# google/libultrahdr

Hardware: AMD Instinct MI355X
Metric: Mpixels/s encode+decode (API-1 P010+YUV420, 4K), device-resident round trip (higher is better)
Workload: dtype f32; 1 GPU; API-1 3840x2160 round trip per step: encode (P010 HLG + YCbCr420 -> two-pass 3-ch gain map at scale 1, FDCT q95, Huffman: two JPEG scans) + decode (Huffman, IDCT, applyGainMap -> RGBA_F16 linear); frames resident in HBM

## Files before the change

libultrahdr_amd/csrc/api_context.cpp:

```cpp
#include "api_internal.h"

#include <sys/mman.h>
#include <mutex>
#include <algorithm>

namespace uhdr_api {
uhdr_error_info_t ensure(DeviceBuf& b, size_t bytes) {
  if (b.cap >= bytes) return ok_status();
  if (b.p) (void)hipFree(b.p);
  b.p = nullptr;
  b.cap = 0;
  size_t want = bytes + (bytes >> 3) + 256;
  HIP_TRY(hipMalloc(&b.p, want));
  b.cap = want;
  return ok_status();
}


size_t bytes_per_sample(int fmt) {
  switch (fmt) {
    case UHDR_IMG_FMT_24bppYCbCrP010:
    case UHDR_IMG_FMT_30bppYCbCr444: return 2;
    case UHDR_IMG_FMT_24bppRGB888: return 3;
    case UHDR_IMG_FMT_32bppRGBA8888:
// ... 484 lines not shown
  if (c->tab_cap[slot] < bytes) {
    HIP_TRY(hipStreamSynchronize(c->stream));
    if (c->h_tab[slot]) (void)hipHostFree(c->h_tab[slot]);
    if (c->d_tab[slot]) (void)hipFree(c->d_tab[slot]);
    c->h_tab[slot] = nullptr; c->d_tab[slot] = nullptr; c->tab_cap[slot] = 0;
    HIP_TRY(hipHostMalloc((void**)&c->h_tab[slot], bytes, hipHostMallocDefault));
    HIP_TRY(hipMalloc((void**)&c->d_tab[slot], bytes));
    if (!c->tab_ev[slot]) HIP_TRY(hipEventCreateWithFlags(&c->tab_ev[slot], hipEventDisableTiming));
    c->tab_cap[slot] = bytes;
  }
  memcpy(c->h_tab[slot], t.data(), bytes);
  HIP_TRY(hipMemcpyAsync(c->d_tab[slot], c->h_tab[slot], bytes, hipMemcpyHostToDevice, c->stream));
  HIP_TRY(hipEventRecord(c->tab_ev[slot], c->stream));
  c->tab_key[slot] = key;
  *d_out = c->d_tab[slot];
  return ok_status();
}
}


const char* uhdr_hip_version(void) { return "libuhdr_hip 0.3 (gfx950; reference libultrahdr 2.0.2 hot path)"; }

int uhdr_hip_device_count(void) {
  int n = 0;
  if (hipGetDeviceCount(&n) != hipSuccess) return 0;
  return n;
}

int uhdr_hip_current_device(void) {
  int d = -1;
  if (hipGetDevice(&d) != hipSuccess) return -1;
  return d;
}

uhdr_hip_ctx_t* uhdr_hip_create(int device, uhdr_error_info_t* err) {
  auto fail = [&](const char* what, hipError_t e) -> uhdr_hip_ctx_t* {
    if (err) *err = err_status(UHDR_CODEC_ERROR, "uhdr_hip_create: %s failed: %s (no CPU fallback exists behind this library)",
                               what, hipGetErrorString(e));
    return nullptr;
  };
  if (err) *err = ok_status();
  int n = 0;
  hipError_t e = hipGetDeviceCount(&n);
  if (e != hipSuccess || n == 0) return fail("hipGetDeviceCount", e == hipSuccess ? hipErrorNoDevice : e);
  if (device < 0) {
    e = hipGetDevice(&device);
    if (e != hipSuccess) return fail("hipGetDevice", e);
  }
  if (device >= n) return fail("device index", hipErrorInvalidDevice);
  e = hipSetDevice(device);
  if (e != hipSuccess) return fail("hipSetDevice", e);
  uhdr_hip_ctx* c = new uhdr_hip_ctx();
  c->device = device;
  e = hipStreamCreateWithFlags(&c->own_stream, hipStreamNonBlocking);
  if (e != hipSuccess) { delete c; return fail("hipStreamCreate", e); }
  c->stream = c->own_stream;
  uhdr_error_info_t st = upload_lut(&c->d_srgb, host::srgb_inv_oetf_lut(), c->stream);
  if (st.error_code != UHDR_CODEC_OK) {
    if (err) *err = st;
    (void)hipStreamDestroy(c->own_stream);
    delete c;
    return nullptr;
  }
  return c;
}

void uhdr_hip_destroy(uhdr_hip_ctx_t* c) {
  if (!c) return;
  (void)hipSetDevice(c->device);
  (void)hipStreamSynchronize(c->stream);
  for (auto& e : c->prof_entries) { (void)hipEventDestroy(e.a); (void)hipEventDestroy(e.b); }
  float* luts[] = {c->d_srgb, c->d_hlg_inv, c->d_pq_inv, c->d_hlg_oetf, c->d_pq_oetf, c->d_hlg_inv_ootf, (float*)c->d_math,
                   c->d_hlg_buckets, c->d_pq_buckets, c->d_hlg_buckets_pre, c->d_pq_buckets_pre};
  for (float* p : luts) if (p) (void)hipFree(p);
  for (int i = 0; i < kTableSlots; i++) {
    if (c->h_tab[i]) (void)hipHostFree(c->h_tab[i]);
    if (c->d_tab[i]) (void)hipFree(c->d_tab[i]);
    if (c->tab_ev[i]) (void)hipEventDestroy(c->tab_ev[i]);
  }
  for (auto& b : c->scratch) if (b.p) (void)hipFree(b.p);
  for (auto& b : c->jpg) if (b.p) (void)hipFree(b.p);
  for (auto& b : c->enc) if (b.p) (void)hipFree(b.p);
  for (auto& r : c->resident) if (r.buf.p) (void)hipFree(r.buf.p);
  if (c->pending.buf.p) (void)hipFree(c->pending.buf.p);
  if (c->pending.tmp.p) (void)hipFree(c->pending.tmp.p);
  if (c->minmax.p) (void)hipFree(c->minmax.p);
  if (c->d_coef_src) (void)hipFree(c->d_coef_src);
  if (c->d_huff) (void)hipFree(c->d_huff);
  if (c->d_srgb8) (void)hipFree(c->d_srgb8);
  for (float* q : c->d_lin10) if (q) (void)hipFree(q);
  for (auto& g : c->gain_tabs) if (g.d) (void)hipFree(g.d);
  uhdr_hip_comm_destroy(c);
  aux_worker_destroy(c);
  if (c->aux) uhdr_hip_destroy(c->aux);
  if (c->exchange.p) (void)hipFree(c->exchange.p);
  if (c->affine.p) (void)hipFree(c->affine.p);
  if (c->d_srgb_of_byte) (void)hipFree(c->d_srgb_of_byte);
  if (c->h_mm) (void)hipHostFree(c->h_mm);
  if (c->aux_ev) (void)hipEventDestroy(c->aux_ev);
  if (c->aux_ev2) (void)hipEventDestroy(c->aux_ev2);
  if (c->md_ev) (void)hipEventDestroy(c->md_ev);
  if (c->md_stream) (void)hipStreamDestroy(c->md_stream);
  if (c->h_flags) (void)hipHostFree(c->h_flags);
  if (c->pin.p) (void)hipHostFree(c->pin.p);
  if (c->pin.ev) (void)hipEventDestroy(c->pin.ev);
  if (c->huff_tabs.dev.p) (void)hipFree(c->huff_tabs.dev.p);
  if (c->own_stream) (void)hipStreamDestroy(c->own_stream);
  delete c;
}

int uhdr_hip_recycle(uhdr_hip_ctx_t* c, size_t keep_bytes) {
  if (!c) return -1;
  (void)hipSetDevice(c->device);
  (void)hipStreamSynchronize(c->stream);
  uhdr_hip_resident_forget(c);
  uhdr_hip_resident_begin(c);
  uhdr_hip_resident_end(c);
  c->sticky = ok_status();
  for (auto& h : c->huff_hint) h = uhdr_hip_ctx::HuffHint();
  c->stats = uhdr_hip_stats_t();
  c->deferred_md.valid = false;
  std::vector<DeviceBuf*> bufs;
  for (auto& b : c->scratch) bufs.push_back(&b);
  for (auto& b : c->jpg) bufs.push_back(&b);
  for (auto& b : c->enc) bufs.push_back(&b);
  for (auto& r : c->resident) bufs.push_back(&r.buf);
  bufs.push_back(&c->pending.buf);
  bufs.push_back(&c->pending.tmp);
  size_t total = c->pin.cap;
  for (DeviceBuf* b : bufs) total += b->p ? b->cap : 0;
  std::sort(bufs.begin(), bufs.end(), [](const DeviceBuf* a, const DeviceBuf* b) { return (a->p ? a->cap : 0) > (b->p ? b->cap : 0); });
  for (DeviceBuf* b : bufs) {
    if (total <= keep_bytes) break;
    if (!b->p) continue;
    (void)hipFree(b->p);
    total -= b->cap;
    b->p = nullptr;
    b->cap = 0;
  }
  if (total > keep_bytes && c->pin.p) {
    if (c->pin.ev_pending && c->pin.ev) (void)hipEventSynchronize(c->pin.ev);
    (void)hipHostFree(c->pin.p);
    c->pin.p = nullptr;
    c->pin.cap = c->pin.off = 0;
    c->pin.ev_pending = false;
  }
  if (c->aux) (void)uhdr_hip_recycle(c->aux, keep_bytes);
  return c->device;
}

uhdr_error_info_t uhdr_hip_set_stream(uhdr_hip_ctx_t* c, void* hip_stream) {
  if (!c) return err_status(UHDR_CODEC_INVALID_PARAM, "received nullptr for uhdr_hip context");
  HIP_TRY(hipStreamSynchronize(c->stream));
  c->stream = hip_stream ? (hipStream_t)hip_stream : c->own_stream;
  return ok_status();
}

void* uhdr_hip_get_stream(uhdr_hip_ctx_t* c) { return c ? (void*)c->stream : nullptr; }

uhdr_error_info_t uhdr_hip_synchronize(uhdr_hip_ctx_t* c) {
  if (!c) return err_status(UHDR_CODEC_INVALID_PARAM, "received nullptr for uhdr_hip context");
  HIP_TRY(hipStreamSynchronize(c->stream));
  return ok_status();
}

void uhdr_hip_get_stats(uhdr_hip_ctx_t* c, uhdr_hip_stats_t* out) {
  if (!out) return;
  if (!c) { memset(out, 0, sizeof *out); return; }
  *out = c->stats;
}

namespace {
std::mutex g_seam_mu;
std::vector<uhdr_hip_seam_stage_t> g_seam_rows;
unsigned long long g_seam_seq = 0;
void seam_dump_at_exit() {
  const char* path = getenv("UHDR_HIP_SEAM_STATS_FILE");
  FILE* f = path ? fopen(path, "w") : nullptr;
// ... 176 lines not shown
```

libultrahdr_amd/csrc/api_entropy.cpp:

```cpp
#include "api_internal.h"

#include <condition_variable>
#include <functional>
#include <mutex>

uhdr_error_info_t uhdr_api::check_scan(const uhdr_hip_jpeg_scan_t* sc, bool need_coef, int* mcus_per_row, int* mcu_rows, int* blocks_per_mcu) {
  if (!sc) return err_status(UHDR_CODEC_INVALID_PARAM, "received nullptr for the scan description");
  if (sc->num_components != 1 && sc->num_components != 3)
    return err_status(UHDR_CODEC_INVALID_PARAM, "a scan has 1 or 3 components, received %d", sc->num_components);
  if (sc->w == 0 || sc->h == 0 || sc->w > 65535 || sc->h > 65535)
    return err_status(UHDR_CODEC_INVALID_PARAM, "image dimensions %ux%u are outside JPEG's 1..65535", sc->w, sc->h);
  int hmax = 1, vmax = 1, bpm = 0;
  for (int i = 0; i < sc->num_components; i++) {
    const int hs = sc->num_components == 1 ? 1 : sc->h_samp[i], vs = sc->num_components == 1 ? 1 : sc->v_samp[i];
    if (hs < 1 || hs > 2 || vs < 1 || vs > 2) return err_status(UHDR_CODEC_INVALID_PARAM, "component %d: sampling factors %dx%d not in {1, 2}", i, hs, vs);
    if (hs > hmax) hmax = hs;
    if (vs > vmax) vmax = vs;
    bpm += hs * vs;
    if (need_coef && (!sc->coef[i] || ((uintptr_t)sc->coef[i] & 15)))
      return err_status(UHDR_CODEC_INVALID_PARAM, "coefficient buffer %d is null or not 16-byte aligned", i);
    if (sc->blocks_w[i] < 1 || sc->blocks_h[i] < 1) return err_status(UHDR_CODEC_INVALID_PARAM, "component %d: empty block grid", i);
  }
  if (sc->num_components == 1) {
    *mcus_per_row = sc->blocks_w[0];
// ... 32 lines not shown


uhdr_error_info_t uhdr_hip_huffman_encode_dev(uhdr_hip_ctx_t* c, const uhdr_hip_jpeg_scan_t* sc, uint8_t* out, size_t out_capacity,
                                              size_t* out_bytes) {
  if (!c) return err_status(UHDR_CODEC_INVALID_PARAM, "received nullptr for uhdr_hip context");
  if (!out || !out_bytes) return err_status(UHDR_CODEC_INVALID_PARAM, "received nullptr for the output buffer or size");
  int mpr = 0, mrows = 0, bpm = 0;
  UHDR_TRY(check_scan(sc, true, &mpr, &mrows, &bpm));
  const bool stream = sc->restart_interval == 0;
  if (!stream && (sc->restart_interval < 1 || sc->restart_interval > 65535 || sc->restart_interval * bpm > 64))
    return err_status(UHDR_CODEC_UNSUPPORTED_FEATURE, "restart_interval must be 0 (no markers) or in 1..%d for %d blocks per MCU (one wavefront "
                      "encodes one restart interval of at most 64 blocks); received %d", 64 / bpm, bpm, sc->restart_interval);
  if (stream && 2 * bpm > 64) return err_status(UHDR_CODEC_UNSUPPORTED_FEATURE, "%d blocks per MCU: outside the HIP path", bpm);
  HIP_TRY(hipSetDevice(c->device));
  if (!c->d_huff) {
    std::vector<uint32_t> blob(host::jpeg_huff_code_tables());
    blob.resize((size_t)host::kHuffTabWords + 16);
    memcpy(blob.data() + host::kHuffTabWords, host::jpeg_zigzag_to_natural(), 64);
    HIP_TRY(hipMalloc((void**)&c->d_huff, blob.size() * sizeof(uint32_t)));
    HIP_TRY(hipMemcpyAsync(c->d_huff, blob.data(), blob.size() * sizeof(uint32_t), hipMemcpyHostToDevice, c->stream));
    HIP_TRY(hipStreamSynchronize(c->stream));
  }
  HuffArgs a;
  memset(&a, 0, sizeof a);
  a.ncomp = sc->num_components;
  for (int i = 0; i < a.ncomp; i++) {
    a.coef[i] = sc->coef[i];
    a.bw[i] = sc->blocks_w[i]; a.bh[i] = sc->blocks_h[i];
    a.hs[i] = a.ncomp == 1 ? 1 : sc->h_samp[i]; a.vs[i] = a.ncomp == 1 ? 1 : sc->v_samp[i];
  }
  a.mcus_per_row = mpr;
  a.total_mcus = mpr * mrows;
  a.ri = stream ? huff_stream_segment_mcus(bpm) : sc->restart_interval;
  a.blocks_per_mcu = bpm;
  a.nseg = (a.total_mcus + a.ri - 1) / a.ri;
  a.tables = c->d_huff;
  a.zigzag = (const uint8_t*)(c->d_huff + host::kHuffTabWords);
  if (stream) {
    if (out_capacity > 0xFFFFFFF0u) out_capacity = 0xFFFFFFF0u;
    HuffStream t;
    memset(&t, 0, sizeof t);
    t.raw_words = ((uint64_t)out_capacity + 3) / 4 + 1;
    const uint64_t worst_words = (uint64_t)a.total_mcus * bpm * 52 + 2;
    if (t.raw_words > worst_words) t.raw_words = worst_words;
    const int nchunks = huff_stuff_chunks(t.raw_words * 4u);
    UHDR_TRY(ensure(c->scratch[4], (size_t)t.raw_words * 4));
    UHDR_TRY(ensure(c->scratch[5], ((size_t)a.nseg + 2) * sizeof(uint64_t) + (4 + (size_t)a.nseg + (size_t)nchunks) * sizeof(uint32_t)));
    t.raw = (uint32_t*)c->scratch[4].p;
    t.seg_start = (uint64_t*)c->scratch[5].p;
    uint64_t* d_total = t.seg_start + (size_t)a.nseg + 1;
    t.meta = (uint32_t*)(d_total + 1);
    t.seg_bits = t.meta + 4;
    uint32_t* chunk_counts = t.seg_bits + a.nseg;
    {
      ProfScope ps(c, "huffman_encode");
      HIP_TRY(launch_huffman_encode_stream(a, t, chunk_counts, d_total, out, (uint64_t)out_capacity, c->stream));
    }
    c->stats.entropy_encode_stream++;
    if (!c->h_flags) HIP_TRY(hipHostMalloc((void**)&c->h_flags, 64 * sizeof(uint32_t), hipHostMallocDefault));
    uint32_t* hp = c->h_flags + 48;
    HIP_TRY(hipMemcpyAsync(hp, d_total, sizeof(uint64_t) + 4 * sizeof(uint32_t), hipMemcpyDeviceToHost, c->stream));
    HIP_TRY(wait_stream(c));
    uint64_t total = 0;
    uint32_t meta[4] = {0, 0, 0, 0};
    memcpy(&total, hp, sizeof total);
    memcpy(meta, hp + 2, sizeof meta);
    if (meta[2]) return err_status(UHDR_CODEC_INVALID_PARAM, "coefficients outside the baseline range (DC difference beyond 11 bits / AC beyond 10 bits)");
    const uint64_t raw_bytes = ((((uint64_t)meta[1] << 32) | meta[0]) + 7) / 8;
    if (raw_bytes > t.raw_words * 4u) total = raw_bytes + raw_bytes / 64 + 64;
    *out_bytes = (size_t)total;
    if (total > out_capacity)
      return err_status(UHDR_CODEC_MEM_ERROR, "entropy-coded data needs %llu bytes, the output buffer holds %zu", (unsigned long long)total, out_capacity);
    return ok_status();
  }
  a.slot_stride = huff_slot_stride();
  UHDR_TRY(ensure(c->scratch[4], (size_t)a.nseg * a.slot_stride));
  const size_t meta = (size_t)a.nseg * sizeof(uint32_t) + 16 + ((size_t)a.nseg + 1) * sizeof(uint64_t) + 16;
  UHDR_TRY(ensure(c->scratch[5], meta));
  a.slots = (uint8_t*)c->scratch[4].p;
  uint64_t* offsets = (uint64_t*)c->scratch[5].p;
  uint32_t* status = (uint32_t*)(offsets + (size_t)a.nseg + 1);
  a.seg_bytes = status + 2;
  {
    ProfScope ps(c, "huffman_encode");
    HIP_TRY(launch_huffman_encode(a, offsets, status, out, (uint64_t)out_capacity, c->stream));
  }
  c->stats.entropy_encode_intervals++;
  uint64_t total = 0;
  uint32_t bad = 0;
  HIP_TRY(hipMemcpyAsync(&total, offsets + a.nseg, sizeof total, hipMemcpyDeviceToHost, c->stream));
  HIP_TRY(hipMemcpyAsync(&bad, status, sizeof bad, hipMemcpyDeviceToHost, c->stream));
  HIP_TRY(wait_stream(c));
  if (bad) return err_status(UHDR_CODEC_INVALID_PARAM, "coefficients outside the baseline range (DC difference beyond 11 bits / AC beyond 10 bits)");
  *out_bytes = (size_t)total;
  if (total > out_capacity)
    return err_status(UHDR_CODEC_MEM_ERROR, "entropy-coded data needs %llu bytes, the output buffer holds %zu", (unsigned long long)total, out_capacity);
  return ok_status();
}

static bool make_dec_table(const uint8_t bits[17], const uint8_t vals[256], HuffDecTable* t) {
  memset(t, 0, sizeof *t);
  int nsym = 0;
  for (int l = 1; l <= 16; l++) nsym += bits[l];
  if (nsym > 256) return false;
  int code = 0, k = 0;
  for (int l = 1; l <= 16; l++) {
// ... 508 lines not shown
      if (settled && rst_sync && ((fl[1] & 14u) != 0 || fl[9] != (uint32_t)(a.nseg - 1) || fl[0] != fl[16] || fl[7] != fl[17])) {
        for (int i = 0; i < a.ncomp; i++) HIP_TRY(hipMemsetAsync(a.coef[i], 0, zero_bytes[i], c->stream));
        coef_zeroed = true;
      } else if (settled) {
        if (fl[1] & 8u) return err_status(UHDR_CODEC_INVALID_PARAM, "corrupt entropy-coded data (the scan ends before its last block)");
        if (fl[1] & 2u) return err_status(UHDR_CODEC_INVALID_PARAM, "corrupt entropy-coded data (undefined Huffman code or a run past the end of a block)");
        sync_done = true;
      } else {
        if (a.nseg == 1 && !c->huff_serial_ok && data_bytes > (256u << 10)) {
          c->stats.entropy_decode_declined++;
          return err_status(UHDR_CODEC_UNSUPPORTED_FEATURE, "the parallel entropy decode did not settle in %d rounds; %zu bytes on one lane would take longer than the CPU", max_rounds, data_bytes);
        }
        for (int i = 0; i < a.ncomp; i++) HIP_TRY(hipMemsetAsync(a.coef[i], 0, zero_bytes[i], c->stream));
        coef_zeroed = true;
      }
    }
  }
  if (sync_done) {
    c->stats.entropy_decode_parallel++;
    return ok_status();
  }
  if (a.nseg == 1 && !c->huff_serial_ok && data_bytes > (256u << 10)) {
    c->stats.entropy_decode_declined++;
    return err_status(UHDR_CODEC_UNSUPPORTED_FEATURE, "a %zu-byte scan without restart markers that the parallel decoder does not take (Huffman tables outside its two-level form)", data_bytes);
  }
  if (!coef_zeroed)
    for (int i = 0; i < a.ncomp; i++) HIP_TRY(hipMemsetAsync(a.coef[i], 0, zero_bytes[i], c->stream));
  HIP_TRY(hipMemsetAsync(a.status, 0, 16, c->stream));
  {
    ProfScope ps(c, "huffman_decode");
    HIP_TRY(launch_huffman_decode(a, counts, starts, ends, c->stream));
  }
  if (a.nseg == 1) c->stats.entropy_decode_single_lane++;
  else c->stats.entropy_decode_intervals++;
  uint32_t st[2] = {0, 0};
  HIP_TRY(hipMemcpyAsync(st, a.status, sizeof st, hipMemcpyDeviceToHost, c->stream));
  HIP_TRY(wait_stream(c));
  if (st[1] != (uint32_t)(a.nseg - 1))
    return err_status(UHDR_CODEC_INVALID_PARAM, "found %u restart markers, a restart interval of %d MCUs over %d MCUs needs %d", st[1], a.ri,
                      a.total_mcus, a.nseg - 1);
  if (st[0] & 4u) return err_status(UHDR_CODEC_INVALID_PARAM, "restart markers out of sequence");
  if (st[0] & 2u) return err_status(UHDR_CODEC_INVALID_PARAM, "corrupt entropy-coded data (undefined Huffman code or a run past the end of a block)");
  return ok_status();
}

uhdr_error_info_t uhdr_api::aux_context(uhdr_hip_ctx* c, uhdr_hip_ctx** out) {
  if (!c->aux) {
    uhdr_error_info_t e = ok_status();
    c->aux = uhdr_hip_create(c->device, &e);
    if (!c->aux) return e.error_code != UHDR_CODEC_OK ? e : err_status(UHDR_CODEC_ERROR, "could not create the auxiliary context");
  }
  c->aux->prof = c->prof;
  c->aux->huff_serial_ok = c->huff_serial_ok;
  *out = c->aux;
  return ok_status();
}
void uhdr_api::aux_merge(uhdr_hip_ctx* c) {
  if (!c->aux) return;
  uhdr_hip_ctx* x = c->aux;
  c->stats.entropy_decode_parallel += x->stats.entropy_decode_parallel;
  c->stats.entropy_decode_intervals += x->stats.entropy_decode_intervals;
  c->stats.entropy_decode_single_lane += x->stats.entropy_decode_single_lane;
  c->stats.entropy_decode_declined += x->stats.entropy_decode_declined;
  c->stats.entropy_encode_stream += x->stats.entropy_encode_stream;
  c->stats.entropy_encode_intervals += x->stats.entropy_encode_intervals;
  x->stats = uhdr_hip_stats_t();
  for (auto& e : x->prof_entries) c->prof_entries.push_back(e);
  x->prof_entries.clear();
}

struct AuxWorker {
  static constexpr int kSpinUs = 300;
  std::thread th;
  std::mutex mu;
  std::condition_variable cv;
  std::function<void()> job;
  std::atomic<int> state{0};
  std::atomic<bool> busy{false};
  static bool spin_until(const std::function<bool()>& pred, int us) {
    const auto t0 = std::chrono::steady_clock::now();
    while (!pred()) {
      if (std::chrono::steady_clock::now() - t0 > std::chrono::microseconds(us)) return pred();
#if defined(__x86_64__)
      __builtin_ia32_pause();
#endif
    }
    return true;
  }
  AuxWorker() {
    th = std::thread([this] {
      for (;;) {
        if (!spin_until([this] { return state.load(std::memory_order_acquire) != 0; }, kSpinUs)) {
          std::unique_lock<std::mutex> lk(mu);
          cv.wait(lk, [this] { return state.load(std::memory_order_acquire) != 0; });
        }
        if (state.load(std::memory_order_acquire) == 2) return;
        std::function<void()> j;
        {
          std::lock_guard<std::mutex> lk(mu);
          j = std::move(job);
          state.store(0, std::memory_order_release);
        }
        j();
        {
          std::lock_guard<std::mutex> lk(mu);
          busy.store(false, std::memory_order_release);
// ... 108 lines not shown
```

libultrahdr_amd/csrc/api_internal.h:

```cpp
#ifndef UHDR_HIP_API_INTERNAL_H
#define UHDR_HIP_API_INTERNAL_H

#pragma GCC visibility push(default)
#include "uhdr_hip.h"
#pragma GCC visibility pop

#include <cfloat>
#include <chrono>
#include <cmath>
#include <cstdarg>
#include <cstdio>
#include <cstring>
#include <atomic>
#include <functional>
#include <map>
#include <memory>
#include <string>
#include <thread>
#include <vector>
#include "exact_math.h"
#include "host_tables.h"
#include "uhdr_types.h"
#include "rccl_bind.h"

// ... 24 lines not shown
                        "HIP error '%s' at %s:%d", hipGetErrorString(e_), __FILE__, __LINE__); \
  } while (0)
#define UHDR_TRY(expr)                                 \
  do {                                                 \
    uhdr_error_info_t s_ = (expr);                     \
    if (s_.error_code != UHDR_CODEC_OK) return s_;     \
  } while (0)

struct DbgClock {
  bool on;
  std::chrono::steady_clock::time_point t0;
  DbgClock() : on(getenv("UHDR_HIP_CLOCK_DEBUG") != nullptr), t0(std::chrono::steady_clock::now()) {}
  void mark(const char* what) const {
    if (on) fprintf(stderr, "uhdr_hip:   [%7.1f us] %s\n", std::chrono::duration<double, std::micro>(std::chrono::steady_clock::now() - t0).count(), what);
  }
};

struct ProfEntry {
  hipEvent_t a, b;
  std::string family;
};

constexpr int kTableSlots = 4;

struct DeviceBuf {
  void* p = nullptr;
  size_t cap = 0;
};

struct uhdr_hip_ctx {
  int device = 0;
  hipStream_t own_stream = nullptr;
  hipStream_t stream = nullptr;
  float* d_srgb = nullptr;
  float* d_hlg_inv = nullptr;
  float* d_pq_inv = nullptr;
  float* d_hlg_oetf = nullptr;
  float* d_pq_oetf = nullptr;
  float* d_hlg_buckets = nullptr;
  float* d_pq_buckets = nullptr;
  float* d_hlg_buckets_pre = nullptr;
  float* d_pq_buckets_pre = nullptr;
  float* d_hlg_inv_ootf = nullptr;
  double* d_math = nullptr;
  float* h_tab[kTableSlots] = {};
  float* d_tab[kTableSlots] = {};
  size_t tab_cap[kTableSlots] = {};
  hipEvent_t tab_ev[kTableSlots] = {};
  std::string tab_key[kTableSlots];
  int tab_next = 0;
  DeviceBuf scratch[8];
  uhdr_hip_stats_t stats = {};
  bool huff_serial_ok = true;
  DeviceBuf enc[3];
  uhdr_hip_ctx* aux = nullptr;
  struct AuxWorker* aux_worker = nullptr;
  DeviceBuf jpg[6];
  struct Resident {
    DeviceBuf buf;
    bool valid = false;
    uhdr_img_fmt_t fmt = UHDR_IMG_FMT_UNSPECIFIED;
    unsigned int w = 0, h = 0;
    const void* host[3] = {};
    unsigned int host_stride[3] = {};
    size_t off[3] = {};
    unsigned int dev_stride[3] = {};
    unsigned int prows[3] = {}, pcols[3] = {};
    bool host_unwritten = false;
    bool adopted = false;
    void* adopt_dst = nullptr;
    unsigned int adopt_stride = 0, adopt_w = 0, adopt_h = 0;
    bool adopt_expand = false;
  } resident[2];
  struct HuffHint { uint32_t sub_bits = 0, bits_per_block = 0; } huff_hint[16];
  struct HuffTabCache {
    bool valid = false, fast_ok = false;
    uint8_t key[4 * (17 + 256)] = {};
    DeviceBuf dev;
  } huff_tabs;
  struct PinArena {
    void* p = nullptr;
    size_t cap = 0, off = 0;
    hipEvent_t ev = nullptr;
    bool ev_pending = false;
  } pin;
  uint32_t* h_flags = nullptr;
  bool resident_on = false;
  bool resident_lazy = false;
  uhdr_error_info_t sticky = {};
  unsigned int resident_next = 0;
  struct PendingCopy {
    DeviceBuf buf;
    bool on = false;
    size_t off = 0, pitch = 0, dst_pitch = 0;
    unsigned int w = 0, h = 0, bps = 0;
    bool expand = false;
    void* dst = nullptr;
    DeviceBuf tmp;
  } pending;
  struct MallEntry { const void* p; uint64_t stamp; };
  std::vector<MallEntry> mall;
  uint64_t mall_clock = 0;
  DeviceBuf minmax;
  uint32_t* d_huff = nullptr;
  CoefSrc* d_coef_src = nullptr;
  unsigned int coef_src_next = 0;
// ... 94 lines not shown
```

libultrahdr_amd/csrc/huffman_encode.hip:

```cpp
#include "lds_copy.h"
#include "wg_scan.h"
#include "uhdr_types.h"

namespace uhdr {
namespace {

constexpr int kSegBlocks = 64;
constexpr int kWordsPerBlock = 52;
constexpr int kCoefRow = 33;

__device__ __forceinline__ uint32_t wave_incl_scan(uint32_t v, uint32_t lane) {
#pragma unroll
  for (int d = 1; d < 64; d <<= 1) {
    const uint32_t y = (uint32_t)__shfl_up((int)v, d, 64);
    if (lane >= (uint32_t)d) v += y;
  }
  return v;
}

__device__ __forceinline__ uint64_t zigzag_nonzero_map(const uint32_t* s_coef, uint32_t zz_of_lane, uint32_t lane) {
  uint64_t mine = 0;
  const uint32_t word = zz_of_lane >> 1, sh = (zz_of_lane & 1u) * 16u;
#pragma unroll 4
  for (uint32_t b = 0; b < (uint32_t)kSegBlocks; b++) {
// ... 316 lines not shown
      else pred = s_dc[(int)lane - bpm + hs * vs - 1];
    }
    const uint32_t* dct = s_tab + (c ? (16 + 256) : 0);
    const uint32_t* act = dct + 16;
    const int diff = dcv - pred;
    const uint64_t nz = zigzag_nonzero_map(s_coef, s_zz[lane], lane);
    uint32_t len = 0, oob = 0;
    if (emits) walk_block(dct, act, diff, real, crow, s_zz, nz, oob, [&](uint32_t, uint32_t n) { len += n; });
    const uint32_t incl = wave_incl_scan(len, lane);
    const uint32_t total_bits = (uint32_t)__shfl((int)incl, 63, 64);
    if constexpr (PASS == 0) {
      const bool bad = __builtin_amdgcn_ballot_w64(oob != 0) != 0;
      if (lane == 0) t.seg_bits[seg] = bad ? kBadCoef : total_bits;
    } else {
      const uint32_t phase = (uint32_t)(start & 31u);
      if (phase + total_bits > kCapBits) continue;
      const uint32_t nwords = (phase + total_bits + 31u) >> 5;
      for (uint32_t i = lane; i < nwords + 1u; i += 64) s_bits[i] = 0u;
      __syncthreads();
      if (emits) {
        const uint32_t off = phase + incl - len;
        uint64_t acc = 0;
        uint32_t cnt = off & 31u, w = off >> 5;
        walk_block(dct, act, diff, real, crow, s_zz, nz, oob, [&](uint32_t code, uint32_t n) {
          acc = (acc << n) | (uint64_t)code;
          cnt += n;
          if (cnt >= 32u) {
            cnt -= 32u;
            atomicOr(&s_bits[w++], (uint32_t)(acc >> cnt));
          }
        });
        if (cnt) atomicOr(&s_bits[w], (uint32_t)(acc << (32u - cnt)));
      }
      __syncthreads();
      const uint64_t end_bit = start + total_bits;
      if (seg == a.nseg - 1 && lane == 0 && (end_bit & 7u)) {
        const uint32_t e = phase + total_bits, pad = 8u - (e & 7u), pos = e & 31u;
        s_bits[e >> 5] |= ((1u << pad) - 1u) << (32u - pos - pad);
      }
      __syncthreads();
      const uint64_t w0 = start >> 5;
      const uint32_t tail = (phase + total_bits) & 31u;
      for (uint32_t i = lane; i < nwords; i += 64) {
        if (w0 + i >= t.raw_words) break;
        const uint32_t v = __builtin_bswap32(s_bits[i]);
        const bool shared = (i == 0 && phase != 0) || (i == nwords - 1 && tail != 0);
        if (shared) atomicOr(&t.raw[w0 + i], v);
        else t.raw[w0 + i] = v;
      }
    }
  }
}

template <int NT = 1024, typename Sink>
__device__ __forceinline__ uint64_t wg_scan_tiles(const uint32_t* __restrict__ v, int n, uint32_t* s_val , uint64_t* s_sum , Sink sink) {
  const int tid = (int)threadIdx.x;
  uint64_t carry = 0;
  for (int base = 0; base < n; base += 8 * NT) {
    uint32_t ld[8];
#pragma unroll
    for (int j = 0; j < 8; j++) ld[j] = v[min(base + j * NT + tid, n - 1)];
#pragma unroll
    for (int j = 0; j < 8; j++) s_val[j * NT + tid] = base + j * NT + tid < n ? ld[j] : 0u;
    __syncthreads();
    uint32_t x[8];
    uint64_t sum = 0;
#pragma unroll
    for (int j = 0; j < 8; j++) { x[j] = s_val[tid * 8 + j]; sum += x[j]; }
    uint64_t sc[1] = {sum}, all[1];
    wg_incl_scan<NT, 1>(sc, s_sum, all);
    uint64_t run = carry + sc[0] - sum;
#pragma unroll
    for (int j = 0; j < 8; j++) {
      const int i = base + tid * 8 + j;
      if (i < n) sink(i, x[j], run);
      run += x[j];
    }
    carry += all[0];
  }
  return carry;
}

constexpr int kStreamScanThreads = 256;
__global__ __launch_bounds__(kStreamScanThreads) void huff_stream_scan_kernel(const uint32_t* __restrict__ seg_bits, int nseg, const HuffStream t) {
  __shared__ uint32_t s_val[8 * kStreamScanThreads];
  __shared__ uint64_t s_sum[kStreamScanThreads / 64];
  __shared__ uint32_t s_bad;
  const int tid = (int)threadIdx.x;
  if (tid == 0) s_bad = 0;
  __syncthreads();
  bool bad = false;
  uint32_t big = 0;
  const uint64_t total = wg_scan_tiles<kStreamScanThreads>(seg_bits, nseg, s_val, s_sum, [&](int i, uint32_t n, uint64_t run) {
    bad |= n >= kRetry;
    big += (n < kRetry && n + 32u > (uint32_t)(kSegBlocks * kWordsSmall) * 32u) ? 1u : 0u;
    t.seg_start[i] = run;
    if ((run >> 5) < t.raw_words) t.raw[run >> 5] = 0u;
  });
  if (bad) atomicOr(&s_bad, 1u);
  if (big) atomicAdd(&s_bad, big << 1);
  __syncthreads();
  if (tid == kStreamScanThreads - 1) {
    t.seg_start[nseg] = total;
    if ((total >> 5) < t.raw_words) t.raw[total >> 5] = 0u;
    t.meta[0] = (uint32_t)total;
    t.meta[1] = (uint32_t)(total >> 32);
// ... 55 lines not shown
  if ((uint64_t)blockIdx.x * kStuffChunk >= nraw) return;
  const uint64_t base = (uint64_t)blockIdx.x * kStuffChunk + threadIdx.x * 16u;
  uint4 v = make_uint4(0, 0, 0, 0);
  uint32_t nv = 0;
  if (base < nraw) {
    v = raw_load16(t, base);
    nv = (uint32_t)min((uint64_t)16, nraw - base);
  }
  const uint32_t mask = ff_mask16(v, nv), nff = (uint32_t)__builtin_popcount(mask);
  const uint32_t lane = threadIdx.x & 63, wv = threadIdx.x >> 6;
  const uint32_t incl = wave_incl_scan(nff, lane);
  if (lane == 63) s_wave[wv] = incl;
  __syncthreads();
  uint32_t before = chunk_base[blockIdx.x] + incl - nff;
  for (uint32_t k = 0; k < wv; k++) before += s_wave[k];
  uint64_t pos = base + before;
  if (mask == 0 && nv == 16 && pos + 16 <= cap) {
    uint8_t* d = out + pos;
    __builtin_memcpy(d, &v.x, 4);
    __builtin_memcpy(d + 4, &v.y, 4);
    __builtin_memcpy(d + 8, &v.z, 4);
    __builtin_memcpy(d + 12, &v.w, 4);
    return;
  }
  const uint32_t w[4] = {v.x, v.y, v.z, v.w};
  for (uint32_t k = 0; k < nv; k++) {
    const uint32_t b = (w[k >> 2] >> (8u * (k & 3u))) & 0xffu;
    if (pos < cap) out[pos] = (uint8_t)b;
    pos++;
    if (b == 0xffu) {
      if (pos < cap) out[pos] = 0;
      pos++;
    }
  }
}

}

uint32_t huff_slot_stride() { return (uint32_t)(kSegBlocks * kWordsPerBlock * 4 * 2); }

hipError_t launch_huffman_encode(const HuffArgs& a, uint64_t* offsets, uint32_t* status, uint8_t* out, uint64_t cap, hipStream_t s) {
  int grid = a.nseg < 8192 ? a.nseg : 8192;
  const int per = a.ri * a.blocks_per_mcu, groups = per > 32 ? 1 : 64 / per;
  const int nwseg = (a.nseg + groups - 1) / groups;
  hipLaunchKernelGGL((huff_encode_kernel<kWordsSmall, false>), dim3(nwseg < 8192 ? nwseg : 8192), dim3(64), 0, s, a);
  hipLaunchKernelGGL((huff_encode_kernel<kWordsPerBlock, true>), dim3(grid < 2048 ? grid : 2048), dim3(64), 0, s, a);
  hipLaunchKernelGGL(huff_offsets_kernel, dim3(1), dim3(1024), 0, s, a.seg_bytes, a.nseg, offsets, status);
  hipLaunchKernelGGL(huff_gather_kernel, dim3(grid), dim3(256), 0, s, a.slots, a.slot_stride, a.seg_bytes, offsets, a.nseg, out, cap);
  return hipGetLastError();
}


int huff_stream_segment_mcus(int blocks_per_mcu) { return kSegBlocks / blocks_per_mcu - 1; }
int huff_stuff_chunks(uint64_t raw_bytes) { return (int)((raw_bytes + kStuffChunk - 1) / kStuffChunk); }

hipError_t launch_huffman_encode_stream(const HuffArgs& a, const HuffStream& t, uint32_t* chunk_counts, uint64_t* out_bytes, uint8_t* out, uint64_t cap,
                                        hipStream_t s) {
  const int grid = a.nseg < 16384 ? a.nseg : 16384;
  const int nchunks = huff_stuff_chunks(t.raw_words * 4u);
  hipLaunchKernelGGL((huff_stream_kernel<1, 0>), dim3(grid), dim3(64), 0, s, a, t);
  hipLaunchKernelGGL(huff_stream_scan_kernel, dim3(1), dim3(kStreamScanThreads), 0, s, (const uint32_t*)t.seg_bits, a.nseg, t);
  hipLaunchKernelGGL((huff_stream_kernel<kWordsSmall, 1>), dim3(grid), dim3(64), 0, s, a, t);
  hipLaunchKernelGGL((huff_stream_kernel<kWordsPerBlock, 2>), dim3(grid < 2048 ? grid : 2048), dim3(64), 0, s, a, t);
  hipLaunchKernelGGL(huff_stuff_count_kernel, dim3(nchunks), dim3(256), 0, s, t, chunk_counts);
  hipLaunchKernelGGL(huff_stuff_scan_kernel, dim3(1), dim3(kStreamScanThreads), 0, s, chunk_counts, nchunks, t, out_bytes);
  hipLaunchKernelGGL(huff_stuff_scatter_kernel, dim3(nchunks), dim3(256), 0, s, t, (const uint32_t*)chunk_counts, out, cap);
  return hipGetLastError();
}

}
```

libultrahdr_amd/csrc/uhdr_types.h:

```cpp
#pragma once
#include <hip/hip_runtime.h>
#include <stdint.h>

#include "device_math.h"
#include "uhdr_hip.h"

namespace uhdr {

struct ImageView {
  const void* p[3];
  uint32_t stride[3];
  uint32_t w, h;
  int fmt;
  int range;
};
struct ImageViewMut {
  void* p[3];
  uint32_t stride[3];
  uint32_t w, h;
  int fmt;
  int range;
};

constexpr int kSrgbN = 1024;
// ... 186 lines not shown
hipError_t launch_base_blocks(const ImageView& yuv420, const Mat3* c, const uint16_t* qt_luma, const uint16_t* qt_chroma, int16_t* const coef[3],
                              hipStream_t s);
hipError_t launch_selftest(int which, unsigned long long* out, uint32_t arg0, uint32_t arg1, uint32_t seed, const double* math_tab, const AffineDev* dev,
                           hipStream_t s);
int gen_partials_count(const GenParams& p);
hipError_t launch_encode_api0_fused(const FusedParams& p, bool two_pass, int* grid_out, hipStream_t s);
hipError_t launch_tone_map(const ToneMapParams& p, hipStream_t s);
hipError_t launch_transform_yuv(const YuvXformParams& p, hipStream_t s);
hipError_t launch_rgb_to_ycbcr(const RgbToYcbcrParams& p, hipStream_t s);
struct FdctEdge {
  int on, w, h, col_mode, fill, mcu_rows;
};
hipError_t launch_fdct_quant(const uint8_t* plane, size_t stride, int bw, int bh,
                             const uint16_t* qt_host, int16_t* coef, hipStream_t s, const FdctEdge* edge = nullptr);

hipError_t launch_fdct_quant_rgb(const uint8_t* rgb, size_t pitch, int bpp, int bw, int bh, const uint16_t* qt_luma_host,
                                 const uint16_t* qt_chroma_host, int16_t* coef_y, int16_t* coef_cb, int16_t* coef_cr, hipStream_t s, int vw = 0,
                                 int vh = 0);
hipError_t launch_repack(int mode, const void* src, size_t src_pitch, void* dst, size_t dst_pitch, uint32_t w, uint32_t h,
                         hipStream_t s);
struct EffectPlane {
  const void* src;
  void* dst;
  uint32_t elem;
  uint32_t src_w, src_h, src_stride;
  uint32_t dst_w, dst_h, dst_stride;
  uint32_t mode;
  uint32_t a0, a1;
};
hipError_t launch_effect_plane(const EffectPlane& p, hipStream_t s);

struct HuffArgs {
  const int16_t* coef[3];
  int bw[3], bh[3];
  int hs[3], vs[3];
  int ncomp;
  int mcus_per_row, total_mcus;
  int ri;
  int blocks_per_mcu;
  int nseg;
  const uint32_t* tables;
  const uint8_t* zigzag;
  uint8_t* slots;
  uint32_t slot_stride;
  uint32_t* seg_bytes;
};
uint32_t huff_slot_stride();
struct HuffStream {
  uint32_t* seg_bits;
  uint64_t* seg_start;
  uint32_t* raw;
  uint64_t raw_words;
  uint32_t* meta;
};
int huff_stream_segment_mcus(int blocks_per_mcu);
int huff_stuff_chunks(uint64_t raw_bytes);
hipError_t launch_huffman_encode_stream(const HuffArgs& a, const HuffStream& t, uint32_t* chunk_counts, uint64_t* out_bytes, uint8_t* out, uint64_t cap,
                                        hipStream_t s);
hipError_t launch_huffman_encode(const HuffArgs& a, uint64_t* offsets, uint32_t* status, uint8_t* out, uint64_t cap, hipStream_t s);

struct HuffDecTable {
  uint16_t lut[512];
  int maxcode[18];
  int valoff[17];
  uint8_t vals[256];
};
struct HuffDecArgs {
  const uint8_t* data;
  uint32_t nbytes;
  const uint32_t* starts;
  const uint32_t* ends;
  int nseg, ri, total_mcus, mcus_per_row, ncomp;
  int bw[3], bh[3], hs[3], vs[3];
  int16_t* coef[3];
  const HuffDecTable* tabs;
  const uint8_t* zigzag;
  uint32_t* status;
};
constexpr int kHuffL2Max = 16;
struct HuffFastTable {
  uint16_t l1[512];
  uint16_t l2[kHuffL2Max][128];
};
constexpr int kHuffValWords = 512 + kHuffL2Max * 128;
constexpr int kHuffPairBits = 10, kHuffPairWords = 1 << kHuffPairBits;
constexpr int kHuffL2Total = 32;
constexpr int kHuffPairBlobWords = 4 * kHuffPairWords + kHuffL2Total * 128 / 2;
constexpr int kHuffPairValBlobWords = 8 * kHuffPairWords + kHuffL2Total * 128 / 2;
struct HuffSyncArgs {
  const uint8_t* clean;
  uint32_t nbytes;
  const uint32_t* nstuffed;
  uint32_t sub_bits;
  uint64_t* state[2];
  uint8_t* changed[2];
  uint32_t* nblk;
  uint32_t* scan_tmp;
  uint32_t* flags;
  int* dcd;
  uint32_t total_blocks;
  int blocks_per_mcu, ncomp, mcus_per_row;
  int bw[3], bh[3], hs[3], vs[3], first_blk[3];
  uint8_t comp_of[16];
  int16_t* coef[3];
  const HuffFastTable* ftabs;
  const HuffFastTable* ttabs;
  const uint32_t* vtabs;
  const uint32_t* ptabs;
// ... 60 lines not shown
```

Measured before the change: 11660 Mpixels/s.

## Encode Huffman segments in one walk into slots, then place bits after scan

Replaces the two-pass stream Huffman encode, which first walks every block to count bits and then walks again to emit them at the scanned offsets. Each wave now walks its segment once: it counts bit lengths, packs the bits in LDS and writes them to a per-segment slot buffer. A place kernel then shifts each slot into the bitstream at the scanned offset. This adds a slot buffer in device memory, falls back to the two-pass route when that allocation fails, and adds extra global traffic for the slot copies.

Result: faster. 12110 Mpixels/s (median of 6 runs) (+3.9%).

```diff
diff --git a/libultrahdr_amd/csrc/api_context.cpp b/libultrahdr_amd/csrc/api_context.cpp
--- a/libultrahdr_amd/csrc/api_context.cpp
+++ b/libultrahdr_amd/csrc/api_context.cpp
@@ -560,6 +560,12 @@
   if (e != hipSuccess) return fail("hipSetDevice", e);
   uhdr_hip_ctx* c = new uhdr_hip_ctx();
   c->device = device;
+  {
+    const char* e = getenv("UHDR_HIP_HUFF_TWO_PASS");
+    c->huff_two_pass = e && atoi(e) != 0;
+    e = getenv("UHDR_HIP_HUFF_ROUTE_LOG");
+    c->huff_route_log = e && atoi(e) != 0;
+  }
   e = hipStreamCreateWithFlags(&c->own_stream, hipStreamNonBlocking);
   if (e != hipSuccess) { delete c; return fail("hipStreamCreate", e); }
   c->stream = c->own_stream;
@@ -589,6 +595,7 @@
   for (auto& b : c->scratch) if (b.p) (void)hipFree(b.p);
   for (auto& b : c->jpg) if (b.p) (void)hipFree(b.p);
   for (auto& b : c->enc) if (b.p) (void)hipFree(b.p);
+  if (c->huff_slots.p) (void)hipFree(c->huff_slots.p);
   for (auto& r : c->resident) if (r.buf.p) (void)hipFree(r.buf.p);
   if (c->pending.buf.p) (void)hipFree(c->pending.buf.p);
   if (c->pending.tmp.p) (void)hipFree(c->pending.tmp.p);
@@ -628,10 +635,12 @@
   for (auto& h : c->huff_hint) h = uhdr_hip_ctx::HuffHint();
   c->stats = uhdr_hip_stats_t();
   c->deferred_md.valid = false;
+  c->huff_slots_refused = 0;
   std::vector<DeviceBuf*> bufs;
   for (auto& b : c->scratch) bufs.push_back(&b);
   for (auto& b : c->jpg) bufs.push_back(&b);
   for (auto& b : c->enc) bufs.push_back(&b);
+  bufs.push_back(&c->huff_slots);
   for (auto& r : c->resident) bufs.push_back(&r.buf);
   bufs.push_back(&c->pending.buf);
   bufs.push_back(&c->pending.tmp);
diff --git a/libultrahdr_amd/csrc/api_entropy.cpp b/libultrahdr_amd/csrc/api_entropy.cpp
--- a/libultrahdr_amd/csrc/api_entropy.cpp
+++ b/libultrahdr_amd/csrc/api_entropy.cpp
@@ -108,6 +108,19 @@
     t.meta = (uint32_t*)(d_total + 1);
     t.seg_bits = t.meta + 4;
     uint32_t* chunk_counts = t.seg_bits + a.nseg;
+    if (!c->huff_two_pass) {
+      const size_t need = huff_stream_slot_bytes(a.nseg);
+      if (c->huff_slots.cap >= need || !c->huff_slots_refused || need < c->huff_slots_refused) {
+        if (ensure(c->huff_slots, need).error_code == UHDR_CODEC_OK) {
+          t.slots = (uint32_t*)c->huff_slots.p;
+        } else {
+          (void)hipGetLastError();
+          c->huff_slots_refused = need;
+          fprintf(stderr, "uhdr_hip: no device memory for %zu bytes of Huffman segment slots: marker-less scans of that size take the two-pass route\n", need);
+        }
+      }
+    }
+    if (c->huff_route_log) fprintf(stderr, "uhdr_hip: huffman_encode stream route=%s nseg=%d\n", t.slots ? "one_walk" : "two_pass", a.nseg);
     {
       ProfScope ps(c, "huffman_encode");
       HIP_TRY(launch_huffman_encode_stream(a, t, chunk_counts, d_total, out, (uint64_t)out_capacity, c->stream));
@@ -722,6 +735,8 @@
   }
   c->aux->prof = c->prof;
   c->aux->huff_serial_ok = c->huff_serial_ok;
+  c->aux->huff_route_log = c->huff_route_log;
+  c->aux->huff_two_pass = c->huff_two_pass;
   *out = c->aux;
   return ok_status();
 }
diff --git a/libultrahdr_amd/csrc/api_internal.h b/libultrahdr_amd/csrc/api_internal.h
--- a/libultrahdr_amd/csrc/api_internal.h
+++ b/libultrahdr_amd/csrc/api_internal.h
@@ -100,6 +100,10 @@
   DeviceBuf scratch[8];
   uhdr_hip_stats_t stats = {};
   bool huff_serial_ok = true;
+  DeviceBuf huff_slots;
+  bool huff_two_pass = false;
+  bool huff_route_log = false;
+  size_t huff_slots_refused = 0;
   DeviceBuf enc[3];
   uhdr_hip_ctx* aux = nullptr;
   struct AuxWorker* aux_worker = nullptr;
diff --git a/libultrahdr_amd/csrc/huffman_encode.hip b/libultrahdr_amd/csrc/huffman_encode.hip
--- a/libultrahdr_amd/csrc/huffman_encode.hip
+++ b/libultrahdr_amd/csrc/huffman_encode.hip
@@ -392,6 +392,130 @@
   }
 }
 
+constexpr int kWalkSegs = 4;
+constexpr int kSlotWords = kSegBlocks * kWordsSmall;
+__device__ __forceinline__ void wave_sync() {
+  __builtin_amdgcn_fence(__ATOMIC_SEQ_CST, "wavefront");
+  __builtin_amdgcn_wave_barrier();
+}
+__global__ __launch_bounds__(64 * kWalkSegs) void huff_stream_walk_kernel(const HuffArgs a, const HuffStream t) {
+  __shared__ __attribute__((aligned(16))) uint32_t s_tab[2 * (16 + 256)];
+  __shared__ uint32_t s_coef_all[kWalkSegs][kSegBlocks * kCoefRow];
+  __shared__ uint32_t s_bits_all[kWalkSegs][kSlotWords];
+  __shared__ uint8_t s_zz[64];
+  const uint32_t lane = threadIdx.x & 63u, wv = threadIdx.x >> 6;
+  copy_words_to_lds<4>(s_tab, a.tables, 2 * (16 + 256), threadIdx.x, 64 * kWalkSegs);
+  if (threadIdx.x < 64) s_zz[threadIdx.x] = a.zigzag[threadIdx.x];
+  __syncthreads();
+  uint32_t* s_coef = s_coef_all[wv];
+  uint32_t* s_bits = s_bits_all[wv];
+  const int bpm = a.blocks_per_mcu;
+  const int mcu_local = (int)lane / bpm, k_in_mcu = (int)lane - mcu_local * bpm;
+  int c = 0, kk = k_in_mcu;
+  if (a.ncomp > 1) {
+    while (c < a.ncomp - 1 && kk >= a.hs[c] * a.vs[c]) { kk -= a.hs[c] * a.vs[c]; c++; }
+  }
+  const int hs = a.ncomp > 1 ? a.hs[c] : 1, vs = a.ncomp > 1 ? a.vs[c] : 1;
+  const int yi = kk / hs, xi = kk - yi * hs;
+  const int pred_lane = (kk > 0 ? (int)lane - 1 : (int)lane - bpm + hs * vs - 1) & 63;
+  const uint32_t* dct = s_tab + (c ? (16 + 256) : 0);
+  const uint32_t* act = dct + 16;
+  const uint32_t zz_of_lane = s_zz[lane];
+  uint32_t* crow = s_coef + lane * kCoefRow;
+  for (int seg = (int)blockIdx.x * kWalkSegs + (int)wv; seg < a.nseg; seg += (int)gridDim.x * kWalkSegs) {
+    wave_sync();
+    const int mcu = seg * a.ri + mcu_local - 1;
+    const bool valid = mcu_local <= a.ri && mcu >= 0 && mcu < a.total_mcus;
+    const bool emits = valid && mcu_local >= 1;
+    const int mcu_c = valid ? mcu : 0;
+    const int my = mcu_c / a.mcus_per_row, mx = mcu_c - my * a.mcus_per_row;
+    const int by = my * vs + yi, bx = mx * hs + xi;
+    const bool real = valid && by < a.bh[c] && bx < a.bw[c];
+    int dc0 = 0;
+    if (real) {
+      const uint4* src = (const uint4*)(a.coef[c] + ((size_t)by * a.bw[c] + bx) * 64);
+      if (emits) {
+        uint4 q[8];
+#pragma unroll
+        for (int i = 0; i < 8; i++) q[i] = src[i];
+#pragma unroll
+        for (int i = 0; i < 8; i++) { crow[4 * i] = q[i].x; crow[4 * i + 1] = q[i].y; crow[4 * i + 2] = q[i].z; crow[4 * i + 3] = q[i].w; }
+        dc0 = (int)(int16_t)(q[0].x & 0xffffu);
+      } else {
+        dc0 = (int)(int16_t)(*(const uint32_t*)src & 0xffffu);
+      }
+    }
+    const uint64_t real_mask = __builtin_amdgcn_ballot_w64(real);
+    const int up1 = __shfl_up(dc0, 1, 64), up2 = __shfl_up(dc0, 2, 64), up3 = __shfl_up(dc0, 3, 64);
+    int dcv = dc0;
+    if (valid && !real) {
+      if (k_in_mcu >= 1 && ((real_mask >> (lane - 1)) & 1ull)) dcv = up1;
+      else if (k_in_mcu >= 2 && ((real_mask >> (lane - 2)) & 1ull)) dcv = up2;
+      else if (k_in_mcu >= 3 && ((real_mask >> (lane - 3)) & 1ull)) dcv = up3;
+    }
+    const int pred_v = __shfl(dcv, pred_lane, 64);
+    const int diff = dcv - (emits ? pred_v : 0);
+    wave_sync();
+    const uint64_t nz = zigzag_nonzero_map(s_coef, zz_of_lane, lane);
+    uint32_t len = 0, oob = 0;
+    if (emits) walk_block(dct, act, diff, real, crow, s_zz, nz, oob, [&](uint32_t, uint32_t n) { len += n; });
+    const uint32_t incl = wave_incl_scan(len, lane);
+    const uint32_t total_bits = (uint32_t)__shfl((int)incl, 63, 64);
+    const bool bad = __builtin_amdgcn_ballot_w64(oob != 0) != 0;
+    if (lane == 0) t.seg_bits[seg] = bad ? kBadCoef : total_bits;
+    if (bad || total_bits + 32u > (uint32_t)kSlotWords * 32u) continue;
+    const uint32_t nwords = (total_bits + 31u) >> 5;
+    for (uint32_t i = lane; i < nwords + 1u; i += 64) s_bits[i] = 0u;
+    wave_sync();
+    if (emits) {
+      const uint32_t off = incl - len;
+      uint64_t acc = 0;
+      uint32_t cnt = off & 31u, w = off >> 5;
+      walk_block(dct, act, diff, real, crow, s_zz, nz, oob, [&](uint32_t code, uint32_t n) {
+        acc = (acc << n) | (uint64_t)code;
+        cnt += n;
+        if (cnt >= 32u) {
+          cnt -= 32u;
+          atomicOr(&s_bits[w++], (uint32_t)(acc >> cnt));
+        }
+      });
+      if (cnt) atomicOr(&s_bits[w], (uint32_t)(acc << (32u - cnt)));
+    }
+    wave_sync();
+    uint32_t* slot = t.slots + (size_t)seg * (size_t)kSlotWords;
+    for (uint32_t i = lane; i < nwords; i += 64) slot[i] = s_bits[i];
+  }
+}
+
+constexpr int kPlaceSegs = 4;
+__global__ __launch_bounds__(64 * kPlaceSegs) void huff_stream_place_kernel(int nseg, const HuffStream t) {
+  const uint32_t lane = threadIdx.x & 63u;
+  const int seg = (int)blockIdx.x * kPlaceSegs + (int)(threadIdx.x >> 6);
+  if (seg >= nseg) return;
+  const uint32_t total_bits = t.seg_bits[seg];
+  if (total_bits >= kRetry || total_bits + 32u > (uint32_t)(kSegBlocks * kWordsSmall) * 32u) return;
+  const uint64_t start = t.seg_start[seg];
+  const uint32_t phase = (uint32_t)(start & 31u);
+  const uint32_t nin = (total_bits + 31u) >> 5, nwords = (phase + total_bits + 31u) >> 5;
+  const uint32_t e = phase + total_bits, tail = e & 31u;
+  const bool flush = seg == nseg - 1 && (e & 7u);
+  const uint32_t* slot = t.slots + (size_t)seg * (size_t)(kSegBlocks * kWordsSmall);
+  const uint64_t w0 = start >> 5;
+  for (uint32_t i = lane; i < nwords; i += 64) {
+    if (w0 + i >= t.raw_words) break;
+    const uint32_t cur = i < nin ? slot[i] : 0u, prev = (i > 0 && phase != 0) ? slot[i - 1] : 0u;
+    uint32_t v = __builtin_amdgcn_alignbit(prev, cur, phase);
+    if (flush && i == (e >> 5)) {
+      const uint32_t pad = 8u - (e & 7u);
+      v |= ((1u << pad) - 1u) << (32u - tail - pad);
+    }
+    v = __builtin_bswap32(v);
+    const bool shared = (i == 0 && phase != 0) || (i == nwords - 1 && tail != 0);
+    if (shared) atomicOr(&t.raw[w0 + i], v);
+    else t.raw[w0 + i] = v;
+  }
+}
+
 template <int NT = 1024, typename Sink>
 __device__ __forceinline__ uint64_t wg_scan_tiles(const uint32_t* __restrict__ v, int n, uint32_t* s_val , uint64_t* s_sum , Sink sink) {
   const int tid = (int)threadIdx.x;
@@ -553,15 +677,23 @@
 
 
 int huff_stream_segment_mcus(int blocks_per_mcu) { return kSegBlocks / blocks_per_mcu - 1; }
+size_t huff_stream_slot_bytes(int nseg) { return (size_t)nseg * (size_t)kSlotWords * sizeof(uint32_t); }
 int huff_stuff_chunks(uint64_t raw_bytes) { return (int)((raw_bytes + kStuffChunk - 1) / kStuffChunk); }
 
 hipError_t launch_huffman_encode_stream(const HuffArgs& a, const HuffStream& t, uint32_t* chunk_counts, uint64_t* out_bytes, uint8_t* out, uint64_t cap,
                                         hipStream_t s) {
   const int grid = a.nseg < 16384 ? a.nseg : 16384;
   const int nchunks = huff_stuff_chunks(t.raw_words * 4u);
-  hipLaunchKernelGGL((huff_stream_kernel<1, 0>), dim3(grid), dim3(64), 0, s, a, t);
-  hipLaunchKernelGGL(huff_stream_scan_kernel, dim3(1), dim3(kStreamScanThreads), 0, s, (const uint32_t*)t.seg_bits, a.nseg, t);
-  hipLaunchKernelGGL((huff_stream_kernel<kWordsSmall, 1>), dim3(grid), dim3(64), 0, s, a, t);
+  if (t.slots) {
+    const int wgrid = (grid + kWalkSegs - 1) / kWalkSegs;
+    hipLaunchKernelGGL(huff_stream_walk_kernel, dim3(wgrid), dim3(64 * kWalkSegs), 0, s, a, t);
+    hipLaunchKernelGGL(huff_stream_scan_kernel, dim3(1), dim3(kStreamScanThreads), 0, s, (const uint32_t*)t.seg_bits, a.nseg, t);
+    hipLaunchKernelGGL(huff_stream_place_kernel, dim3((a.nseg + kPlaceSegs - 1) / kPlaceSegs), dim3(64 * kPlaceSegs), 0, s, a.nseg, t);
+  } else {
+    hipLaunchKernelGGL((huff_stream_kernel<1, 0>), dim3(grid), dim3(64), 0, s, a, t);
+    hipLaunchKernelGGL(huff_stream_scan_kernel, dim3(1), dim3(kStreamScanThreads), 0, s, (const uint32_t*)t.seg_bits, a.nseg, t);
+    hipLaunchKernelGGL((huff_stream_kernel<kWordsSmall, 1>), dim3(grid), dim3(64), 0, s, a, t);
+  }
   hipLaunchKernelGGL((huff_stream_kernel<kWordsPerBlock, 2>), dim3(grid < 2048 ? grid : 2048), dim3(64), 0, s, a, t);
   hipLaunchKernelGGL(huff_stuff_count_kernel, dim3(nchunks), dim3(256), 0, s, t, chunk_counts);
   hipLaunchKernelGGL(huff_stuff_scan_kernel, dim3(1), dim3(kStreamScanThreads), 0, s, chunk_counts, nchunks, t, out_bytes);
diff --git a/libultrahdr_amd/csrc/uhdr_types.h b/libultrahdr_amd/csrc/uhdr_types.h
--- a/libultrahdr_amd/csrc/uhdr_types.h
+++ b/libultrahdr_amd/csrc/uhdr_types.h
@@ -262,8 +262,10 @@
   uint32_t* raw;
   uint64_t raw_words;
   uint32_t* meta;
+  uint32_t* slots;
 };
 int huff_stream_segment_mcus(int blocks_per_mcu);
+size_t huff_stream_slot_bytes(int nseg);
 int huff_stuff_chunks(uint64_t raw_bytes);
 hipError_t launch_huffman_encode_stream(const HuffArgs& a, const HuffStream& t, uint32_t* chunk_counts, uint64_t* out_bytes, uint8_t* out, uint64_t cap,
                                         hipStream_t s);
```
